# mjiUST/SurfaceNet

Hardware: AMD Instinct MI355X
Metric: voxel-cubes/sec (CVC warp + 3D CNN fwd) at s=32, N_viewpair=2 (higher is better)
Workload: dtype f16x3 (each operand = hi+lo fp16 pair, 3 MFMAs per product, f32 accumulate: fp32-class results; the two correction terms of a product run on one MX-scaled MFMA in the two merge layers (fp6 e2m3 codes) and in the three dilated layers conv4_x (fp8 e4m3 codes); L_inf vs fp64 oracle 3e-5 .. 1.7e-4, asse; 1 GPU; synthetic 2-view 1600x1200, s=32, batch=64 cubes/GPU, N_viewpair=2 (BASELINE.json configs[1]); cubes_per_gpu=64, parallelism=cube-sharded x1

## Files before the change

surfacenet_amd/csrc/conv3d_mfma.h:

```cpp
#pragma once
#include <hip/hip_runtime.h>
#include "mx_format.h"
#include <stdint.h>
#include <type_traits>

constexpr int kRowGap3x3 = 4, kRowGap2D = 4, kRowGapDil2 = 2;
#ifndef SN_TIMING
#define SN_TIMING 0
#endif
#define PW_SB __builtin_amdgcn_sched_barrier(0)

namespace sn {

typedef _Float16 half8 __attribute__((ext_vector_type(8)));
typedef _Float16 half4 __attribute__((ext_vector_type(4)));
typedef float f32x4 __attribute__((ext_vector_type(4)));

constexpr int kMaxSlab = 128;

struct ConvArgs {
    const _Float16 *in;
    _Float16 *out;
    float *out_f32;
    const _Float16 *wpack;
// ... 154 lines not shown
    static constexpr int TX = F4 ? NW * MF : NW * XS, TY = F4 ? 4 : 8, TZ = F4 ? 4 : 8;
    static constexpr int HX = TX + 2 * RX, HY = TY + 2 * R, HZ = TZ + 2 * R;
    static constexpr int HVOX = HX * HY * HZ;
    static constexpr int CS8MAX = CS8;
    static constexpr int SLOTS = CS8 + PADV_;
    static constexpr int VS = SLOTS * 16;
    static constexpr int PCH = PCH_;
    static constexpr int NPL = SPLIT ? 2 : 1;
    static constexpr int NPLM = SPLIT == 1 ? 2 : 1;
    static constexpr int FRAG = 1024 * NPL;
    static constexpr int MFRAG = 1024 * NPLM;
    static_assert(SPLIT < 2 || PCH_ == 2, "f16m8: a weight piece is 2 K-chunks + one MX step");
    static constexpr int MXF = SPLIT == 3 ? 0 : SN_MX_FMT;
    static constexpr int WBUF = PCH * NF * FRAG;
    static constexpr int NTAP = (K2D ? 1 : KS) * KS * KS;
    static constexpr int KOFF_N = NTAP * CS8MAX + 24;
    static constexpr bool PWM = (SPLIT == 3 || (SPLIT == 2 && SN_MX_FMT != 0)) && K2D == 0 && NW_ == 4 && KS == 3 && MF == 8 && PCH_ == 2;
    static constexpr int PW_TABS = 16;
    static constexpr int pw_tab(int kb, int slab, bool last) { return kb * PW_TABS + (last ? 8 : 0) + (slab & 7); }
    static constexpr int pw_xoff(int m) { return (((m >> 2) * HY + (m & 3)) * HZ) * VS; }
    static constexpr int XGAP = DIL == 2 ? kRowGapDil2 : kRowGap3x3;
    static constexpr int xoff_of(int m) { return XGAP == 4 ? pw_xoff(m) : (((m >> 2) * HY + (m & 1) + 4 * ((m >> 1) & 1)) * HZ) * VS; }
    static constexpr bool PTAB = SPLIT < 2 && NW_ == 8 && KS == 3 && PCH_ >= 2 && (K2D == 0 || SPLIT != 0) && !PWM;
    static constexpr int KTAB_N = PWM ? PW_TABS * KOFF_N : (PTAB ? 8 * KOFF_N : KOFF_N);
    static constexpr int NSEG0 = (HVOX * VS + 1023) / 1024;
    static constexpr int NSEG = PWM ? (NSEG0 + NW_ - 1) / NW_ * NW_ : NSEG0;
    static constexpr int XPLANE = NSEG * 1024;
    static constexpr int XBUF = XPLANE * NPL;
#ifndef SN_PW_WB3
#define SN_PW_WB3 0
// ... 144 lines not shown
        static_for<0, HT>([&](auto kc) {
            constexpr int k = decltype(kc)::value;
            const int li = k * C::NW + wave;
            if ((k + 1 < HT || C::NSEG * NPL == HT * C::NW || li < C::NSEG * NPL) && k >= kb && k < ke) {
                const char *base = (NPL > 1 && li >= C::NSEG) ? base0 + 2 * a.in_lo_off : base0;
                const __amdgpu_buffer_rsrc_t rs = __builtin_amdgcn_make_buffer_rsrc((void *)base, (short)0, nrec, 0x00020000);
                dma16_buf(rs, (hword[k] & keep) + (unsigned)toff, xbuf + xb * C::XBUF + li * 1024);
                ++issued;
            }
        });
        return issued;
    };
    auto wg_barrier = [&]() { asm volatile("s_barrier" ::: "memory"); };
    constexpr bool BRIDGE_OK = (PPX && SPLIT == 1) || PPM || PWM;
    constexpr int UM = SPLIT >= 2 ? 8 : 4;
    constexpr int BSTEP = (UM - (C::NTAP * C::CS8MAX) % UM) % UM;
    const bool bridge = BRIDGE_OK && a.bridge != 0;
    auto slab_units = [&](int c8n, int slab, int &o, int &b) {
        const int GU = C::NTAP * c8n;
        o = 0; b = 0;
        if (bridge) {
            o = (slab * ((UM - (GU & (UM - 1))) & (UM - 1))) & (UM - 1);
            b = (slab + 1 == a.nslab) ? 0 : ((UM - ((GU - o) & (UM - 1))) & (UM - 1));
        }
        return GU - o + b;
    };
    auto chunks_of = [&](int c8n, int slab) { int o, b; return (slab_units(c8n, slab, o, b) + 3) >> 2; };
    auto wchunks_of = [&](int c8n, int slab) { int o, b; return SPLIT >= 2 ? (((slab_units(c8n, slab, o, b) + 7) >> 3) << 1) : chunks_of(c8n, slab); };
    const int wchunk0 = wchunks_of(slab_c8_of(0), 0);
    auto write_koff_part = [&](int c8n, int kb, int slab, int t0, int nt) {
        int uo, ub;
        const int own = slab_units(c8n, slab, uo, ub) - ub, nchunk = (own + ub + 3) >> 2;
        int *k = kbuf + (PWM ? C::pw_tab(kb, slab, slab + 1 == a.nslab) : (C::PTAB ? kb * 8 + ((slab + 1 == a.nslab) ? 4 : 0) + (slab & 3) : kb)) * C::KOFF_N;
        for (int g = t0; g < (nchunk + 4) * 4; g += nt) {
            int o = 0;
            if (g < own + ub) {
                const int u = g < own ? g + uo : g - own;
                const int far = g < own ? 0 : (1 - 2 * kb) * C::XBUF;
                const int tap = C::CS8MAX == 1 ? u : u / c8n, c8 = C::CS8MAX == 1 ? 0 : u - tap * c8n;
                const int dz = tap % KS, dy = (tap / KS) % KS, dx = tap / (KS * KS);
                o = ((dx * DIL * C::HY + dy * DIL) * C::HZ + dz * DIL) * C::VS + c8 * 16 + far;
            }
            k[g] = o;
        }
    };
    auto write_koff = [&](int c8n, int kb, int slab) { write_koff_part(c8n, kb, slab, tid, C::NT); };
    auto stage_w = [&](size_t off, int nch, int wbi) {
        const int cnt = nch * NF * NPL;
        const char *src = wsrc0 + off;
        char *dst = wbuf + wbi * C::WBUF;
        for (int i = wave; i < cnt; i += C::NW) dma16(src + (size_t)i * 1024 + lane * 16, dst + i * 1024);
    };

    constexpr bool PMAP = (EPI == EPI_SIDEPOOL);
    static_assert(!PMAP || ((MF == 4 || MF == 8) && NW_ == 8 && K2D == 0), "EPI_SIDEPOOL: 8 waves x 4 (8) fragments over an 8x8x8 (16x8x8) tile");
// ... 102 lines not shown
            const unsigned tab0 = kbuf_a + (unsigned)(C::pw_tab(xb, 0, a.nslab == 1) * (C::KOFF_N * 4));
            int koA;
            lds_read32<0>(koA, tab0);
            lds_read32<16>(pw_koB, tab0);
            lds_read64<0>(pw_k2, tab0 + kq * 4);
            lgkm_wait<0>();
            const unsigned xa = xbuf_a + xb * C::XBUF + (unsigned)xbase[0] + (unsigned)koA, wp0 = wbuf_a + wbi * C::WBUF;
            static_for<0, MF>([&](auto mc) { constexpr int m = decltype(mc)::value; lds_read128<C::xoff_of(m)>(pw_xf[m], xa); });
            static_for<0, NF>([&](auto nc) { constexpr int n = decltype(nc)::value; lds_read128<n * 1024>(pw_wf[n], wp0); });
            lgkm_wait<0>();
        }
        if constexpr (PWM) __builtin_assume(a.nslab >= 1);
        for (int slab = 0; slab < a.nslab; ++slab) {
            const bool last_slab = slab + 1 == a.nslab;
            const int c8n = last_slab ? a.c8_last : C::CS8MAX;
            const int su_o = sl_o, su_b = (UM - ((C::NTAP * c8n - su_o) & (UM - 1))) & ((bridge && !last_slab) ? UM - 1 : 0);
            const int units = C::NTAP * c8n - su_o + su_b;
            const int nchunk = (units + 3) >> 2, wchunk = SPLIT >= 2 ? ((units + 7) >> 3) << 1 : nchunk;
            const int npiece = (nchunk + C::PCH - 1) / C::PCH;
            const int ntile = last_slab ? tile + tstride : tile;
            const bool have_next = ntile < a.total_tiles;
            const int nslab_i = last_slab ? 0 : slab + 1;
            const bool nlast = nslab_i + 1 == a.nslab;
            const int nc8n = nlast ? a.c8_last : C::CS8MAX;
            const int n_o = (bridge && !last_slab) ? (su_o + BSTEP) & (UM - 1) : 0;
            const int n_units = C::NTAP * nc8n - n_o + ((UM - ((C::NTAP * nc8n - n_o) & (UM - 1))) & ((bridge && !nlast) ? UM - 1 : 0));
            const int n_wchunk = SPLIT >= 2 ? ((n_units + 7) >> 3) << 1 : (n_units + 3) >> 2;
            const int nc0 = last_slab ? 0 : c0 + c8n;
            const size_t nwoff = last_slab ? 0 : woff + (size_t)wchunk * NF * C::FRAG;
            if constexpr (!PP && !PWM) { if (have_next) write_koff(nc8n, xb ^ 1, nslab_i); }
            int hdone = 0;

            if constexpr (PWM) {
                static_assert(SPLIT >= 2 && C::PCH == 2 && BUFH && EPI != EPI_SIDEPOOL && C::NSEG % C::NW == 0 && C::XPLANE + C::xoff_of(MF - 1) < 65536,
                              "one-wave-per-SIMD loop: f16m8 3x3x3 kernels");
                long long pws1 = 0;
                constexpr int mxo = 2 * NF * 1024;
                constexpr int WCNT = C::PCH * NF * NPL, WPW = (WCNT + C::NW - 1) / C::NW;
                constexpr int NM = MF * NF;
                constexpr int DSP = (NM - 16) / (WPW + HT / 2) >= 3 ? 3 : 2;
                static_assert(MF + NF <= 16 && 16 + DSP * (WPW + HT / 2 - 1) < NM && 4 + 2 * NF + 15 < NM, "filler schedule exceeds the burst");
                const unsigned tab_a = kbuf_a + (unsigned)(C::pw_tab(xb, slab, last_slab) * (C::KOFF_N * 4));
// ... 167 lines not shown
            if constexpr (PPX) {
                static_assert(C::PCH >= 2 && BUFH && SPLIT < 2 && C::PTAB, "ping-pong loop (f16 / f16x3): at least two chunks per weight piece");
                const unsigned koff_a = kbuf_a + (unsigned)((xb * 8 + (last_slab ? 4 : 0) + (slab & 3)) * (C::KOFF_N * 4));
                const unsigned xslab = xbuf_a + xb * C::XBUF;
                constexpr int NPLM = C::NPLM;
                int ko, ko_n = 0;
                const int bridge_b = su_b;
                lds_read32<0>(ko, koff_a);
                lgkm_wait<0>();
                int p = 0;
                do {
                    const int ch0 = p * C::PCH;
                    const unsigned wp = wbuf_a + wbi * C::WBUF;
                    const int nseg = (nchunk - ch0) < C::PCH ? (nchunk - ch0) : C::PCH;
                    int hnow = 0;
                    static_for<0, C::PCH>([&](auto scc) {
                        constexpr int sc = decltype(scc)::value;
                        if (sc < nseg) {
                            half8 xf[NPLM][MF], wf[NPLM][NF];
                            {
                                const unsigned kos = xslab + (unsigned)ko;
                                constexpr bool XIMM = K2D == 0 && !PMAP && KS == 3 && C::XPLANE + C::xoff_of(MF - 1) < 65536;
                                const unsigned kos0 = (unsigned)xbase[0] + kos;
                                static_for<0, MF>([&](auto mc) {
                                    constexpr int m = decltype(mc)::value;
                                    if constexpr (XIMM) {
                                        lds_read128<C::xoff_of(m)>(xf[0][m], kos0);
                                        if constexpr (SPLIT == 1) lds_read128<C::XPLANE + C::xoff_of(m)>(xf[1][m], kos0);
                                    } else {
                                        lds_read128<0>(xf[0][m], (unsigned)xbase[m] + kos);
                                        if constexpr (SPLIT == 1) {
                                            if constexpr (C::XPLANE < 65536) lds_read128<(C::XPLANE < 65536 ? C::XPLANE : 0)>(xf[1][m], (unsigned)xbase[m] + kos);
                                            else lds_read128<0>(xf[1][m], (unsigned)xbase[m] + kos + C::XPLANE);
                                        }
                                    }
                                });
                                static_for<0, NF>([&](auto nc) {
                                    constexpr int n = decltype(nc)::value;
                                    lds_read128<(sc * NF + n) * C::MFRAG>(wf[0][n], wp);
                                    if constexpr (SPLIT == 1) lds_read128<(sc * NF + n) * C::MFRAG + 1024>(wf[1][n], wp);
                                });
                                lds_read32<0>(ko_n, koff_a + (unsigned)(ch0 + sc + 1) * 16);
                            }
                            if constexpr (sc == 0) {
                                const bool real = (p + 1 < npiece) || have_next;
                                const size_t w_off = (p + 1 < npiece) ? woff + (size_t)(ch0 + C::PCH) * NF * C::FRAG : nwoff;
                                int w_nch = C::PCH;
                                if (p + 1 < npiece) { const int rem = wchunk - (ch0 + C::PCH); if (rem < C::PCH) w_nch = rem; }
                                else { if (n_wchunk < C::PCH) w_nch = n_wchunk; }
                                const char *src = wsrc0 + (real ? w_off : 0);
                                char *dst = wbuf + (wbi ^ 1) * C::WBUF;
                                const int cnt = (real ? w_nch : (wchunk0 < C::PCH ? wchunk0 : C::PCH)) * NF * NPL;
                                constexpr int WPWX = (C::PCH * NF * NPL + C::NW - 1) / C::NW;
                                static_for<0, WPWX>([&](auto kc) {
                                    int i = decltype(kc)::value * C::NW + wave;
                                    i = i < cnt ? i : cnt - 1;
                                    dma16(src + (size_t)i * 1024 + lane * 16, dst + i * 1024);
                                });
                                if (p == 0 && have_next)
                                    hnow = stage_halo_buf(last_slab ? nxt_b : (K2D ? x0 : b), last_slab ? nxt_keep : cur_keep, last_slab ? nxt_toff : cur_toff, nc0, nc8n, xb ^ 1);
                            }
                            const bool pre_bridge = bridge_b > 0 && ch0 + sc == nchunk - 2;
                            if (sc == nseg - 1) {
                                if (!pre_bridge && p + 1 < npiece && hnow == HT) asm volatile("s_waitcnt vmcnt(%0)" ::"i"(HT) : "memory");
                                else if (!pre_bridge && p + 1 < npiece && HT > 1 && hnow == HT - 1) asm volatile("s_waitcnt vmcnt(%0)" ::"i"(HT > 1 ? HT - 1 : 0) : "memory");
                                else asm volatile("s_waitcnt vmcnt(0)" ::: "memory");
                            } else if (pre_bridge) asm volatile("s_waitcnt vmcnt(0)" ::: "memory");
                            lgkm_wait<0>();
                            ko = ko_n;
                            wg_barrier();
                            __builtin_amdgcn_sched_barrier(0);
#pragma unroll
                            for (int n = 0; n < NF; ++n) {
                                if constexpr (SPLIT == 1) {
#pragma unroll
                                    for (int m = 0; m < MF; ++m) acc[m][n] = __builtin_amdgcn_mfma_f32_16x16x32_f16(wf[1][n], xf[0][m], acc[m][n], 0, 0, 0);
#pragma unroll
                                    for (int m = 0; m < MF; ++m) acc[m][n] = __builtin_amdgcn_mfma_f32_16x16x32_f16(wf[0][n], xf[1][m], acc[m][n], 0, 0, 0);
                                }
#pragma unroll
                                for (int m = 0; m < MF; ++m) acc[m][n] = __builtin_amdgcn_mfma_f32_16x16x32_f16(wf[0][n], xf[0][m], acc[m][n], 0, 0, 0);
                            }
                            __builtin_amdgcn_sched_barrier(0);
                            wg_barrier();
// ... 665 lines not shown
```

surfacenet_amd/csrc/sn_api.hip:

```cpp
#include "sn_internal.h"

enum Kind { K_CONV3, K_CONV1, K_DIL3, K_DIL1, K_UP };
struct LayerSpec { const char *name; Kind kind; int cin, cout, act; const char *input; };
static const LayerSpec kSpecs[] = {
    {"conv1_1", K_CONV3, 6, 32, 0, nullptr},       {"conv1_2", K_CONV3, 32, 32, 0, "conv1_1"},    {"conv1_3", K_CONV3, 32, 32, 0, "conv1_2"},
    {"side_op1", K_CONV1, 32, 16, 1, "conv1_3"},
    {"conv2_1", K_CONV3, 32, 80, 0, "conv1_3"},    {"conv2_2", K_CONV3, 80, 80, 0, "conv2_1"},    {"conv2_3", K_CONV3, 80, 80, 0, "conv2_2"},
    {"side_op2", K_CONV1, 80, 16, 1, "conv2_3"},   {"side_op2_deconv", K_UP, 3, 2, 0, nullptr},
    {"conv3_1", K_CONV3, 80, 160, 0, "conv2_3"},   {"conv3_2", K_CONV3, 160, 160, 0, "conv3_1"},  {"conv3_3", K_CONV3, 160, 160, 0, "conv3_2"},
    {"side_op3", K_CONV1, 160, 16, 1, "conv3_3"},  {"side_op3_deconv", K_UP, 5, 4, 0, nullptr},
    {"conv4_1", K_DIL3, 160, 300, 0, "conv3_3"},   {"conv4_2", K_DIL3, 300, 300, 0, "conv4_1"},   {"conv4_3", K_DIL3, 300, 300, 0, "conv4_2"},
    {"side_op4", K_DIL1, 300, 16, 1, "conv4_3"},   {"side_op4_deconv", K_UP, 5, 4, 0, nullptr},
    {"merge_conv_a", K_CONV3, 64, 100, 0, nullptr}, {"merge_conv_b", K_CONV3, 100, 100, 0, "merge_conv_a"}, {"merge_conv3", K_CONV1, 100, 1, 1, "merge_conv_b"},
};
static constexpr int kNumSpecs = sizeof(kSpecs) / sizeof(kSpecs[0]);
static constexpr int kNetParams = 98, kAllParams = 105, kDFeature = 258, kHidden = 100;


static unsigned char fp8_e4m3(float v)
{
    if (v != v) return 0x7f;
    const unsigned char sgn = std::signbit(v) ? 0x80 : 0;
    float a = std::fabs(v);
    if (a >= 448.f) return sgn | 0x7e;
// ... 59 lines not shown
            for (size_t i = (size_t)o * L.cin * ntap; i < (size_t)(o + 1) * L.cin * ntap; ++i) Wn[i] = std::ldexp(Wn[i], row_exp[o]);
    }
    if (ntap == 1) L.w_norm = Wn;
    const float *W = Wn.data();
    auto wat = [&](int o, int c8abs, int j, int tap) -> float {
        const int ci = c8abs * 8 + j;
        return (o < L.cout && ci < L.cin) ? W[((size_t)o * L.cin + ci) * ntap + tap] : 0.f;
    };
    h.clear();
    {
        const int um = split >= 2 ? 8 : 4;
        bool ok = L.bridge && (split == 1 || (split >= 2 && !L.k2d)) && L.ks == 3 && L.slab_c8.size() >= 2 && (ntap * cs8max) % um != 0;
        for (unsigned char c8n : L.slab_c8) ok = ok && c8n == cs8max;
        L.bridge = ok ? 1 : 0;
    }
    const int nslab = (int)L.slab_c8.size();
    auto slab_units = [&](int si, int c8n, int &o, int &b) {
        const int GU = ntap * c8n, um = split >= 2 ? 8 : 4;
        o = 0; b = 0;
        if (L.bridge) { o = (si * ((um - GU % um) % um)) % um; b = (si + 1 == nslab) ? 0 : (um - (GU - o) % um) % um; }
        return GU - o + b;
    };
    if (split < 2) {
        long long chunks = 0;
        for (int si = 0; si < nslab; ++si) { int o, b; chunks += (slab_units(si, L.slab_c8[si], o, b) + 3) / 4; }
        L.wsplit_stride = chunks * nf * 512 * npl;
        h.assign((size_t)L.wsplit_stride * nsplit, (_Float16)0.f);
        for (int ns = 0; ns < nsplit; ++ns) {
            _Float16 *dst = h.data() + (size_t)ns * L.wsplit_stride;
            int c8_0 = 0;
            for (int si = 0; si < nslab; ++si) {
                const int c8n = L.slab_c8[si];
                int uo, ub;
                const int own = slab_units(si, c8n, uo, ub) - ub, nchunk = (own + ub + 3) / 4;
                for (int ch = 0; ch < nchunk; ++ch)
                    for (int f = 0; f < nf; ++f)
                        for (int lane = 0; lane < 64; ++lane) {
                            const int o = (ns * nf + f) * 16 + (lane & 15);
                            const int g = 4 * ch + (lane >> 4);
                            _Float16 *d8 = dst + (((size_t)ch * nf + f) * npl * 64 + lane) * 8;
                            if (g >= own + ub) continue;
                            const int u = g < own ? g + uo : g - own;
                            const int cb = g < own ? c8_0 : c8_0 + c8n;
                            for (int j = 0; j < 8; ++j) {
                                const float w = wat(o, cb + u % c8n, j, u / c8n);
                                const _Float16 hi = (_Float16)w;
                                d8[j] = hi;
                                if (split == 1) d8[512 + j] = (_Float16)(w - (float)hi);
                            }
                        }
                dst += (size_t)nchunk * nf * 512 * npl;
                c8_0 += c8n;
            }
        }
    } else {
        long long pieces = 0;
        for (int si = 0; si < nslab; ++si) { int o, b; pieces += (slab_units(si, L.slab_c8[si], o, b) + 7) / 8; }
        const size_t piece_halfs = (size_t)nf * 2048;
        L.wsplit_stride = pieces * piece_halfs;
        h.assign((size_t)L.wsplit_stride * nsplit, (_Float16)0.f);
// ... 85 lines not shown
        const int oe = out_exp ? out_exp[o] : 0;
        sc[o] = std::ldexp(s, oe - row_exp[o]);
        sh[o] = std::ldexp(beta[o] - mean[o] * s, oe);
        if (!std::isfinite(sc[o]) || !std::isfinite(sh[o]) || (s != 0.f && sc[o] == 0.f))
            return fail(SN_ERR_ARG, "%s: folded BatchNorm scale / shift of output channel %d leaves the fp32 range (gamma %g, inv_std %g, "
                                    "row exponent %d, output exponent %d)", L.name.c_str(), o, gamma[o], inv_std[o], row_exp[o], oe);
    }
    L.macs_per_voxel = (double)L.cin * L.cout * ntap;
    return SN_OK;
}

int pack_conv(sn_ctx *c, PackedConv &L, const ConvEntry &e, const float *W_in, const float *beta, const float *gamma, const float *mean,
              const float *inv_std, const int *in_exp, const int *out_exp)
{
    L = PackedConv();
    L.name = e.name; L.cin = e.cin; L.cout = e.cout; L.act = e.act; L.ks = e.k.ks; L.dil = e.k.dil; L.k2d = e.k.k2d; L.bridge = e.bridge;
    std::vector<_Float16> h;
    std::vector<float> sc, sh;
    int rc;
    if ((rc = pack_conv_host(L, W_in, beta, gamma, mean, inv_std, e.k.nf, e.k.nsplit(e.cout), e.k.cs8max, e.k.split, in_exp, out_exp, h, sc, sh)) != SN_OK) return rc;
    if ((rc = dev_alloc(c, &L.wpack, h.size() + 8192)) != SN_OK) return rc;
    if ((rc = dev_alloc(c, &L.scale, sc.size())) != SN_OK) return rc;
    if ((rc = dev_alloc(c, &L.shift, sh.size())) != SN_OK) return rc;
    HIPCHK(hipMemcpy(L.wpack, h.data(), h.size() * sizeof(_Float16), hipMemcpyHostToDevice));
    HIPCHK(hipMemcpy(L.scale, sc.data(), sc.size() * sizeof(float), hipMemcpyHostToDevice));
    HIPCHK(hipMemcpy(L.shift, sh.data(), sh.size() * sizeof(float), hipMemcpyHostToDevice));
    return SN_OK;
}

static int pack_side_frag(sn_ctx *c, PackedConv &S, int producer_nf)
{
// ... 46 lines not shown
enum Tensor : unsigned char { T_NONE, T_X0, T_A1, T_B1, T_CAT, T_P1, T_A2, T_B2, T_S2, T_P2, T_A3, T_B3, T_A4, T_B4, T_S3, T_S4, T_MA, T_A3_HLC, T_A3_HC, T_COUNT };
static const TensorSpec kTensors[T_COUNT] = {
    {nullptr, 0, 0, MX_ACT, 0},      {&sn_ctx::x0, 0, 8, MX_X0, 0},    {&sn_ctx::a1, 0, 32, MX_ACT, 0},  {&sn_ctx::b1, 0, 32, MX_ACT, 0},  {&sn_ctx::cat, 0, 64, MX_CAT, 0},
    {&sn_ctx::p1, 1, 32, MX_ACT, 0}, {&sn_ctx::a2, 1, 80, MX_ACT, 0},  {&sn_ctx::b2, 1, 80, MX_ACT, 0},  {&sn_ctx::s2, 1, 16, MX_ACT, 0},  {&sn_ctx::p2, 2, 80, MX_ACT, 0},
    {&sn_ctx::a3, 2, 160, MX_ACT, 0}, {&sn_ctx::b3, 2, 160, MX_ACT, 0}, {&sn_ctx::a4, 2, 304, MX_ACT, 0}, {&sn_ctx::b4, 2, 304, MX_ACT, 0}, {&sn_ctx::s3, 2, 16, MX_ACT, 0},
    {&sn_ctx::s4, 2, 16, MX_ACT, 0}, {&sn_ctx::ma, 0, 104, MX_ACT, 0}, {&sn_ctx::a3, 2, 160, MX_ACT, 1}, {&sn_ctx::a3, 2, 160, MX_ACT, 2},
};

template <int SP>
static NetPlan build_plan_t(int tail_m8, int c4_m8)
{
    constexpr int PCH = SP == 2 ? 2 : 4;
    using Conv1 = ConvKernel<3, 1, 8, 2, EPI_STORE, SP, 1, PCH, 8, 0>;
    using Side = ConvKernel<1, 1, 4, 1, EPI_STORE, SP, 5, 2, 4, 0>;
    using Conv23 = ConvKernel<3, 1, 4, 5, EPI_STORE, SP, 1, PCH, 8, 0>;
    using Conv4 = ConvKernel<3, 2, 4, 5, EPI_STORE, SP, 1, 2, 8, 0>;
    static const bool unfused = sn_ab_switch("SN_NO_EPI_FUSION") != nullptr;
    static const bool no_bridge = sn_ab_switch("SN_NO_BRIDGE") != nullptr;
    NetPlan p{SP, tail_m8, c4_m8, {}, {kTensors, kTensors + T_COUNT}, launch_pool<SP>, launch_up3<SP>};
    ConvGeom conv1_3 = ConvKernel<3, 1, 4, 2, EPI_SIDEPOOL, SP, 1, (SP == 2 ? 2 : 7), 8, 0>::geom, side_op1 = Side::geom, conv3_3 = Conv23::geom,
             conv4_1 = Conv4::geom, conv4_2 = conv4_1, conv4_3 = conv4_1,
             merge_a = ConvKernel<3, 1, 4, 7, EPI_STORE, SP, (SP == 0 ? 2 : 1), (SP == 0 ? 4 : 2), 8, 0>::geom,
             merge_b = ConvKernel<3, 1, 4, 7, EPI_FINAL, SP, 1, (SP == 0 ? 4 : 2), 8, 0>::geom;
    Tensor conv3_3_out = T_A3, conv4_1_in = T_A3;
    if constexpr (SP == 1) {
        if (tail_m8 >= 2) {
            conv1_3 = ConvKernel<3, 1, 8, 2, EPI_SIDEPOOL, 1, 1, 4, 8, 0, 0, 2>::geom;
            side_op1 = ConvKernel<1, 1, 4, 1, EPI_STORE, 1, 5, 2, 4, 0, 0, 2>::geom;
            p.up3 = launch_up3<1, 2>;
            merge_a = ConvKernel<3, 1, 8, 7, EPI_STORE, 2, 1, 2, 4, 0>::geom;
            merge_b = ConvKernel<3, 1, 8, 7, EPI_FINAL, 2, 1, 2, 4, 0>::geom;
        }
        if (c4_m8) {
            conv4_1 = conv4_2 = ConvKernel<3, 2, 8, 5, EPI_STORE, 3, 1, 2, 4, 0>::geom;
            conv4_3 = ConvKernel<3, 2, 8, 5, EPI_STORE, 3, 1, 2, 4, 0, 0, 1>::geom;
            if (c4_m8 == 2) conv4_1 = ConvKernel<3, 2, 4, 5, EPI_STORE, 1, 1, 2, 8, 0, 0, 3>::geom;
            else { conv3_3 = ConvKernel<3, 1, 4, 5, EPI_STORE, 1, 1, 4, 8, 0, 0, 4>::geom; conv3_3_out = T_A3_HLC; conv4_1_in = T_A3_HC; }
            for (Tensor t : {T_A3, T_A3_HLC, T_A3_HC, T_A4, T_B4}) p.tens[t].e8 = MX_C4;
        }
    }
    auto add = [&](const char *name, ConvGeom k, Tensor in, Tensor out, Tensor pool_out = T_NONE, const char *pool_tag = nullptr) -> ConvEntry & {
        ConvEntry e{name, 0, 0, 0, k, (k.has_bridge && !no_bridge) ? 1 : 0, in, out, pool_out, pool_tag};
        for (const LayerSpec &sp : kSpecs) if (!strcmp(sp.name, name)) { e.cin = sp.cin; e.cout = sp.cout; e.act = sp.act; }
        p.conv.push_back(e);
        return p.conv.back();
    };
    add("conv1_1", Conv1::geom, T_X0, T_A1);
    add("conv1_2", Conv1::geom, T_A1, T_B1);
    add("conv1_3", unfused ? Conv1::geom : conv1_3, T_B1, unfused ? T_A1 : T_NONE);
    add("side_op1", side_op1, T_A1, T_CAT, T_P1, "pool1");
    add("conv2_1", Conv23::geom, T_P1, T_A2);
    add("conv2_2", Conv23::geom, T_A2, T_B2);
    add("conv2_3", unfused ? Conv23::geom : ConvKernel<3, 1, 4, 5, EPI_SIDEPOOL, SP, 1, PCH, 8, 0>::geom, T_B2, unfused ? T_A2 : T_NONE);
    add("side_op2", Side::geom, T_A2, T_S2, T_P2, "pool2");
    add("conv3_1", Conv23::geom, T_P2, T_A3);
    add("conv3_2", Conv23::geom, T_A3, T_B3);
    add("conv3_3", conv3_3, T_B3, conv3_3_out);
    add("side_op3", Side::geom, T_A3, T_S3);
    add("conv4_1", conv4_1, conv4_1_in, T_A4);
    add("conv4_2", conv4_2, T_A4, T_B4);
    add("conv4_3", conv4_3, T_B4, T_A4);
    add("side_op4", Side::geom, T_A4, T_S4).up3 = true;
    add("merge_conv_a", merge_a, T_CAT, T_MA);
    add("merge_conv_b", merge_b, T_MA, T_NONE);
    return p;
}

static NetPlan build_plan(int split, int tail_m8, int c4_m8)
{
    return split == 2 ? build_plan_t<2>(tail_m8, c4_m8) : (split == 1 ? build_plan_t<1>(tail_m8, c4_m8) : build_plan_t<0>(tail_m8, c4_m8));
}
// ... 1062 lines not shown
    if (bytes > (size_t)info[6]) return fail(SN_ERR_ARG, "sn_debug_tensor: %s holds %lld bytes, %zu asked for", name, info[6], bytes);
    const _Float16 *p = d.a3c ? c->a3c : c->*kTensors[d.buf].buf;
    const size_t own = d.a3c || d.fmt != 4 ? bytes : std::min(bytes, (size_t)info[4] * 2);
    HIPCHK(hipSetDevice(c->device));
    HIPCHK(hipStreamSynchronize(c->stream));
    HIPCHK(hipMemcpy(host, p, own, hipMemcpyDeviceToHost));
    if (bytes > own) HIPCHK(hipMemcpy(static_cast<char *>(host) + own, c->a3c, bytes - own, hipMemcpyDeviceToHost));
    return SN_OK;
}

SN_API int sn_debug_pack_host(int cin, int cout, int ks, int dil, int k2d, int nf, int nsplit, int cs8max, int split, const float *W, const float *beta,
                              const float *gamma, const float *mean, const float *inv_std, unsigned long long *out)
{
    if (!W || !beta || !gamma || !mean || !inv_std || !out) return fail(SN_ERR_ARG, "null argument");
    PackedConv L;
    L.name = "debug"; L.cin = cin; L.cout = cout; L.ks = ks; L.dil = dil; L.k2d = k2d;
    L.bridge = 1;
    std::vector<_Float16> h;
    std::vector<float> sc, sh;
    const int rc = pack_conv_host(L, W, beta, gamma, mean, inv_std, nf, nsplit, cs8max, split, nullptr, nullptr, h, sc, sh);
    if (rc != SN_OK) return rc;
    unsigned long long sum = 0;
    const unsigned char *b = reinterpret_cast<const unsigned char *>(h.data());
    for (size_t i = 0; i < h.size() * sizeof(_Float16); ++i) sum = sum * 1099511628211ull + b[i];
    out[0] = h.size(); out[1] = sc.size(); out[2] = sh.size(); out[3] = sum;
    return SN_OK;
}

SN_API int sn_debug_plan(int net, int mode, int conv4_fp8, char *rows, int cap)
{
    if (!rows || cap < 1 || net < 0 || net > 1) return fail(SN_ERR_ARG, "sn_debug_plan: bad argument");
    sn_ctx st;
    int rc = sn_set_precision(&st, mode), n = 0;
    if (rc == SN_OK && conv4_fp8 >= 0) rc = sn_set_conv4_fp8(&st, conv4_fp8);
    if (rc != SN_OK) return rc;
    for (const ConvEntry &e : net == 0 ? build_plan(st.split, st.tail_m8, st.c4_m8).conv : simil_plan(st.split)) {
        n += snprintf(rows + n, (size_t)(cap - n), "%s %d %d %d %d %d %d %d %d %d %d %d %d\n", e.name, e.cin, e.cout, e.k.ks, e.k.dil, e.k.k2d,
                      e.k.nf, e.k.nsplit(e.cout), e.k.cs8max, e.k.split, e.k.osplit, e.k.epi, e.bridge);
        if (n >= cap) return fail(SN_ERR_ARG, "sn_debug_plan: the rows do not fit %d bytes", cap);
    }
    return SN_OK;
}

SN_API int sn_debug_mx6_encode(float v, int fmt) { return (fmt == 2 || fmt == 3) ? (int)mx6_encode(v, fmt) : -1; }

SN_API int sn_debug_timing(sn_ctx *c, unsigned long long *out, int n_layers, char *names, int names_cap)
{
    if (!c || !out || !c->d_num) return fail(SN_ERR_ARG, "null argument");
    HIPCHK(hipStreamSynchronize(c->stream));
    n_layers = std::min(n_layers, 32);
    HIPCHK(hipMemcpy(out, c->d_num + 2, sizeof(unsigned long long) * 4 * n_layers, hipMemcpyDeviceToHost));
    HIPCHK(hipMemset(c->d_num + 2, 0, sizeof(unsigned) * 32 * 8));
    std::string all;
// ... 51 lines not shown
```

surfacenet_amd/csrc/sn_internal.h:

```cpp
#pragma once
#include <hip/hip_runtime.h>
#include <dlfcn.h>

#include <algorithm>
#include <chrono>
#include <cmath>
#include <condition_variable>
#include <memory>
#include <mutex>
#include <thread>
#include <type_traits>
#include <cstring>
#include <map>
#include <string>
#include <vector>

#include "sn_host.h"
#include "conv3d_mfma.h"
#include "cvc_warp.h"
#include "elementwise.h"

using namespace sn;

#define HIPCHK(expr)                                                                                       \
    do {                                                                                                   \
        hipError_t e_ = (expr);                                                                            \
        if (e_ != hipSuccess) return fail(SN_ERR_HIP, "%s failed: %s (%s:%d)", #expr, hipGetErrorString(e_), __FILE__, __LINE__); \
    } while (0)

struct PackedConv {
    std::string name;
    int cin = 0, cout = 0, ks = 1, dil = 1, act = 0;
    int cin_p = 0;
    int nf = 0, nsplit = 1;
    int cs8max = 4, split = 0, k2d = 0;
    int bridge = 0;
    std::vector<unsigned char> slab_c8;
    long long wsplit_stride = 0;
    _Float16 *wpack = nullptr;
    float *scale = nullptr, *shift = nullptr;
    double macs_per_voxel = 0;
    std::vector<float> w_norm;
    _Float16 *side_frag = nullptr;
};

struct sn_ctx;
enum MxExp : unsigned char { MX_ACT, MX_CAT, MX_X0, MX_C4 };

struct Act { _Float16 *p; long long lo; long long code = 0; MxExp e8 = MX_ACT; };

struct SideFuse { const PackedConv *side; Act side_out; int side_cs, side_coff; Act pool_out; int pool_cs; };

struct ConvGeom {
    int ks, dil, k2d, nf, cs8max, split, osplit, epi;
    bool has_bridge;
    int (*launch)(sn_ctx *c, const PackedConv &L, Act in, int in_cs, Act out, int out_cs, int out_coff, int out_cp, float *out_f32, int B, int D, int DX, const SideFuse *sf);
    int nsplit(int cout) const { return ((cout + 15) / 16 + nf - 1) / nf; }
};

struct ConvEntry {
    const char *name; int cin, cout, act;
    ConvGeom k;
    int bridge;
    unsigned char in = 0, out = 0, pool_out = 0;
    const char *pool_tag = nullptr;
    bool up3 = false;
};
struct TensorSpec { _Float16 *sn_ctx::*buf; int level, ch; MxExp e8; int code; };
struct NetPlan {
    int split = -1, tail_m8 = 0, c4_m8 = 0;
// ... 249 lines not shown
            if (it == c->num_names.end() && c->num_names.size() < 31) c->num_names.push_back(L.name);
            a.status = c->d_num;
            constexpr int OS = OSPLIT < 0 ? SPLIT : OSPLIT;
            if (EPI == EPI_STORE && OS >= 2 && L.act == 0) {
                const _Float16 lim = (_Float16)std::min(60000.f, std::ldexp(OS >= 3 ? 255.875f : (SN_MX_FMT == 2 ? 7.5f : 28.f), a.mx_out_e8 - 127));
                unsigned short bits; memcpy(&bits, &lim, 2);
                a.mx_sat_bits = bits;
            }
            a.status_bit = bit < 31 ? (1u << bit) : (1u << 31);
        }
        a.nslab = (int)L.slab_c8.size();
        if (a.nslab < 1) return fail(SN_ERR_STATE, "%s: no channel slabs", L.name.c_str());
        a.bridge = L.bridge;
        if (L.bridge && !geom.has_bridge)
            return fail(SN_ERR_STATE, "%s: packed with bridge chunks, launched on a kernel without them", L.name.c_str());
        if (C::PWM) {
            for (unsigned char c8n : L.slab_c8)
                if (C::NTAP * c8n < 9) return fail(SN_ERR_STATE, "%s: a channel slab of fewer than two weight pieces", L.name.c_str());
        }
        for (int i = 0; i + 1 < a.nslab; ++i)
            if (L.slab_c8[i] != C::CS8MAX) return fail(SN_ERR_STATE, "%s: channel slab %d holds %d groups, the kernel expects %d in all but the last", L.name.c_str(), i, (int)L.slab_c8[i], C::CS8MAX);
        a.c8_last = L.slab_c8.back();
        const double vox = (double)B * DX * D * D;
        const double bytes = vox * 2.0 * (SPLIT ? 2 : 1) * (L.cin + (EPI == EPI_FINAL ? 2 : (EPI == EPI_SIDEPOOL ? 16 + L.cout / 8.0 : L.cout)));
        ProfScope ps(c, L.name, 2.0 * L.macs_per_voxel * vox, bytes);
        const int resident = std::max(1, c->num_cus * C::WG_PER_CU / L.nsplit);
        dim3 grid((unsigned)std::min(a.total_tiles, resident), (unsigned)L.nsplit);
        hipLaunchKernelGGL((conv3d_f16_mfma<KS, DIL, MF, NF, EPI, SPLIT, CS8, PCH, NW, PADV, K2D, OSPLIT>), grid, dim3(NW * 64), 0, c->stream, a);
        HIPCHK(hipGetLastError());
        return SN_OK;
    }
    static constexpr ConvGeom geom = {KS, DIL, K2D != 0, NF, C::CS8MAX, SPLIT, OSPLIT < 0 ? SPLIT : OSPLIT, EPI,
                                      sn::sn_conv_has_bridge<KS, SPLIT, NW, PCH, NF, K2D, MF>(), &launch};
};

struct TmpDev {
    std::vector<void *> p;
    bool ok = true;
    ~TmpDev() { for (void *q : p) (void)hipFree(q); }
    template <typename T> T *out(size_t count)
    {
        void *q = nullptr;
        if (hipMalloc(&q, std::max<size_t>(count, 1) * sizeof(T)) != hipSuccess) { ok = false; return nullptr; }
        p.push_back(q);
        return static_cast<T *>(q);
    }
    template <typename T> T *up(sn_ctx *c, const T *host, size_t count)
    {
// ... 6 lines not shown
```

Measured before the change: 7412 cubes/s.

## Reorder K stream into tap triples to reuse activation fragments across shifted taps

For split-f16 3x3x3 convs with one 8-channel group per slab, the weight stream is reordered so each piece covers three taps along one axis. The kernel loads the activation register window once per triple and reuses shifted fragments across the three taps instead of re-reading LDS for each tap. The offset table and weight packing are rewritten to match, with a launch-time check that packing order equals kernel order. This trades fewer LDS reads for more registers holding the window (rp array) and 3-chunk pieces.

```diff
diff --git a/surfacenet_amd/csrc/conv3d_mfma.h b/surfacenet_amd/csrc/conv3d_mfma.h
--- a/surfacenet_amd/csrc/conv3d_mfma.h
+++ b/surfacenet_amd/csrc/conv3d_mfma.h
@@ -192,6 +192,10 @@
     static constexpr int MXF = SPLIT == 3 ? 0 : SN_MX_FMT;
     static constexpr int WBUF = PCH * NF * FRAG;
     static constexpr int NTAP = (K2D ? 1 : KS) * KS * KS;
+    static constexpr bool TRI = SPLIT == 1 && NW_ == 8 && KS == 3 && DIL == 1 && K2D == 0 && CS8 == 1 && PCH_ == 3;
+    static constexpr int KORDER = !TRI ? 0 : (EPI == 3  ? 2 : 1);
+    static constexpr int UPG = TRI ? NTAP / 3 : NTAP;
+    static constexpr int CPQ = TRI ? 3 : 1;
     static constexpr int KOFF_N = NTAP * CS8MAX + 24;
     static constexpr bool PWM = (SPLIT == 3 || (SPLIT == 2 && SN_MX_FMT != 0)) && K2D == 0 && NW_ == 4 && KS == 3 && MF == 8 && PCH_ == 2;
     static constexpr int PW_TABS = 16;
@@ -366,10 +370,10 @@
     auto wg_barrier = [&]() { asm volatile("s_barrier" ::: "memory"); };
     constexpr bool BRIDGE_OK = (PPX && SPLIT == 1) || PPM || PWM;
     constexpr int UM = SPLIT >= 2 ? 8 : 4;
-    constexpr int BSTEP = (UM - (C::NTAP * C::CS8MAX) % UM) % UM;
+    constexpr int BSTEP = (UM - (C::UPG * C::CS8MAX) % UM) % UM;
     const bool bridge = BRIDGE_OK && a.bridge != 0;
     auto slab_units = [&](int c8n, int slab, int &o, int &b) {
-        const int GU = C::NTAP * c8n;
+        const int GU = C::UPG * c8n;
         o = 0; b = 0;
         if (bridge) {
             o = (slab * ((UM - (GU & (UM - 1))) & (UM - 1))) & (UM - 1);
@@ -377,7 +381,7 @@
         }
         return GU - o + b;
     };
-    auto chunks_of = [&](int c8n, int slab) { int o, b; return (slab_units(c8n, slab, o, b) + 3) >> 2; };
+    auto chunks_of = [&](int c8n, int slab) { int o, b; return ((slab_units(c8n, slab, o, b) + 3) >> 2) * C::CPQ; };
     auto wchunks_of = [&](int c8n, int slab) { int o, b; return SPLIT >= 2 ? (((slab_units(c8n, slab, o, b) + 7) >> 3) << 1) : chunks_of(c8n, slab); };
     const int wchunk0 = wchunks_of(slab_c8_of(0), 0);
     auto write_koff_part = [&](int c8n, int kb, int slab, int t0, int nt) {
@@ -390,7 +394,9 @@
                 const int u = g < own ? g + uo : g - own;
                 const int far = g < own ? 0 : (1 - 2 * kb) * C::XBUF;
                 const int tap = C::CS8MAX == 1 ? u : u / c8n, c8 = C::CS8MAX == 1 ? 0 : u - tap * c8n;
-                const int dz = tap % KS, dy = (tap / KS) % KS, dx = tap / (KS * KS);
+                int dz = tap % KS, dy = (tap / KS) % KS, dx = tap / (KS * KS);
+                if constexpr (C::KORDER == 1) { dx = u / KS; dy = 0; dz = u % KS; }
+                if constexpr (C::KORDER == 2) { dx = 0; dy = u / KS; dz = u % KS; }
                 o = ((dx * DIL * C::HY + dy * DIL) * C::HZ + dz * DIL) * C::VS + c8 * 16 + far;
             }
             k[g] = o;
@@ -523,9 +529,9 @@
         for (int slab = 0; slab < a.nslab; ++slab) {
             const bool last_slab = slab + 1 == a.nslab;
             const int c8n = last_slab ? a.c8_last : C::CS8MAX;
-            const int su_o = sl_o, su_b = (UM - ((C::NTAP * c8n - su_o) & (UM - 1))) & ((bridge && !last_slab) ? UM - 1 : 0);
-            const int units = C::NTAP * c8n - su_o + su_b;
-            const int nchunk = (units + 3) >> 2, wchunk = SPLIT >= 2 ? ((units + 7) >> 3) << 1 : nchunk;
+            const int su_o = sl_o, su_b = (UM - ((C::UPG * c8n - su_o) & (UM - 1))) & ((bridge && !last_slab) ? UM - 1 : 0);
+            const int units = C::UPG * c8n - su_o + su_b;
+            const int nchunk = ((units + 3) >> 2) * C::CPQ, wchunk = SPLIT >= 2 ? ((units + 7) >> 3) << 1 : nchunk;
             const int npiece = (nchunk + C::PCH - 1) / C::PCH;
             const int ntile = last_slab ? tile + tstride : tile;
             const bool have_next = ntile < a.total_tiles;
@@ -533,8 +539,8 @@
             const bool nlast = nslab_i + 1 == a.nslab;
             const int nc8n = nlast ? a.c8_last : C::CS8MAX;
             const int n_o = (bridge && !last_slab) ? (su_o + BSTEP) & (UM - 1) : 0;
-            const int n_units = C::NTAP * nc8n - n_o + ((UM - ((C::NTAP * nc8n - n_o) & (UM - 1))) & ((bridge && !nlast) ? UM - 1 : 0));
-            const int n_wchunk = SPLIT >= 2 ? ((n_units + 7) >> 3) << 1 : (n_units + 3) >> 2;
+            const int n_units = C::UPG * nc8n - n_o + ((UM - ((C::UPG * nc8n - n_o) & (UM - 1))) & ((bridge && !nlast) ? UM - 1 : 0));
+            const int n_wchunk = SPLIT >= 2 ? ((n_units + 7) >> 3) << 1 : ((n_units + 3) >> 2) * C::CPQ;
             const int nc0 = last_slab ? 0 : c0 + c8n;
             const size_t nwoff = last_slab ? 0 : woff + (size_t)wchunk * NF * C::FRAG;
             if constexpr (!PP && !PWM) { if (have_next) write_koff(nc8n, xb ^ 1, nslab_i); }
@@ -732,12 +738,28 @@
                     const unsigned wp = wbuf_a + wbi * C::WBUF;
                     const int nseg = (nchunk - ch0) < C::PCH ? (nchunk - ch0) : C::PCH;
                     int hnow = 0;
+                    constexpr bool TRI = C::TRI;
+                    constexpr int NP = PMAP ? MF / 2 : 4, NC = MF / NP;
+                    constexpr int AXS = (PMAP ? C::HY * C::HZ : C::HZ) * C::VS, CLS = (PMAP ? C::HZ : C::HY * C::HZ) * C::VS;
+                    static_assert(!TRI || (C::PCH == 3 && C::XPLANE + (NC - 1) * CLS + (NP + 1) * AXS < 65536), "triple order: 3-chunk pieces, immediate offsets");
+                    half8 rp[TRI ? NPLM : 1][TRI ? NC : 1][TRI ? NP + 2 : 1];
                     static_for<0, C::PCH>([&](auto scc) {
                         constexpr int sc = decltype(scc)::value;
-                        if (sc < nseg) {
+                        if (TRI || sc < nseg) {
                             half8 xf[NPLM][MF], wf[NPLM][NF];
                             {
                                 const unsigned kos = xslab + (unsigned)ko;
+                                if constexpr (TRI) {
+                                    const unsigned kos0 = (unsigned)xbase[0] + kos;
+                                    static_for<0, MF>([&](auto mc) {
+                                        constexpr int m = decltype(mc)::value, c = PMAP ? (m & 1) : (m >> 2), q = PMAP ? (m >> 1) : (m & 3);
+                                        constexpr int qn = sc == 0 ? q : NP - 1 + sc;
+                                        if constexpr (sc == 0 || q == 0) {
+                                            lds_read128<c * CLS + qn * AXS>(rp[0][c][qn], kos0);
+                                            lds_read128<C::XPLANE + c * CLS + qn * AXS>(rp[1][c][qn], kos0);
+                                        }
+                                    });
+                                } else {
                                 constexpr bool XIMM = K2D == 0 && !PMAP && KS == 3 && C::XPLANE + C::xoff_of(MF - 1) < 65536;
                                 const unsigned kos0 = (unsigned)xbase[0] + kos;
                                 static_for<0, MF>([&](auto mc) {
@@ -753,12 +775,14 @@
                                         }
                                     }
                                 });
+                                }
                                 static_for<0, NF>([&](auto nc) {
                                     constexpr int n = decltype(nc)::value;
                                     lds_read128<(sc * NF + n) * C::MFRAG>(wf[0][n], wp);
                                     if constexpr (SPLIT == 1) lds_read128<(sc * NF + n) * C::MFRAG + 1024>(wf[1][n], wp);
                                 });
-                                lds_read32<0>(ko_n, koff_a + (unsigned)(ch0 + sc + 1) * 16);
+                                if constexpr (!TRI) lds_read32<0>(ko_n, koff_a + (unsigned)(ch0 + sc + 1) * 16);
+                                else if constexpr (sc == C::PCH - 1) lds_read32<0>(ko_n, koff_a + (unsigned)(p + 1) * 16);
                             }
                             if constexpr (sc == 0) {
                                 const bool real = (p + 1 < npiece) || have_next;
@@ -778,14 +802,19 @@
                                 if (p == 0 && have_next)
                                     hnow = stage_halo_buf(last_slab ? nxt_b : (K2D ? x0 : b), last_slab ? nxt_keep : cur_keep, last_slab ? nxt_toff : cur_toff, nc0, nc8n, xb ^ 1);
                             }
-                            const bool pre_bridge = bridge_b > 0 && ch0 + sc == nchunk - 2;
+                            const bool pre_bridge = bridge_b > 0 && ch0 + sc == nchunk - (TRI ? 4 : 2);
                             if (sc == nseg - 1) {
                                 if (!pre_bridge && p + 1 < npiece && hnow == HT) asm volatile("s_waitcnt vmcnt(%0)" ::"i"(HT) : "memory");
                                 else if (!pre_bridge && p + 1 < npiece && HT > 1 && hnow == HT - 1) asm volatile("s_waitcnt vmcnt(%0)" ::"i"(HT > 1 ? HT - 1 : 0) : "memory");
                                 else asm volatile("s_waitcnt vmcnt(0)" ::: "memory");
                             } else if (pre_bridge) asm volatile("s_waitcnt vmcnt(0)" ::: "memory");
                             lgkm_wait<0>();
-                            ko = ko_n;
+                            if constexpr (!TRI || sc == C::PCH - 1) ko = ko_n;
+                            if constexpr (TRI)
+                                static_for<0, MF>([&](auto mc) {
+                                    constexpr int m = decltype(mc)::value, c = PMAP ? (m & 1) : (m >> 2), q = PMAP ? (m >> 1) : (m & 3);
+                                    xf[0][m] = rp[0][c][q + sc]; xf[NPLM - 1][m] = rp[NPLM - 1][c][q + sc];
+                                });
                             wg_barrier();
                             __builtin_amdgcn_sched_barrier(0);
 #pragma unroll
diff --git a/surfacenet_amd/csrc/sn_api.hip b/surfacenet_amd/csrc/sn_api.hip
--- a/surfacenet_amd/csrc/sn_api.hip
+++ b/surfacenet_amd/csrc/sn_api.hip
@@ -97,16 +97,21 @@
         for (unsigned char c8n : L.slab_c8) ok = ok && c8n == cs8max;
         L.bridge = ok ? 1 : 0;
     }
+    {
+        bool ok = (L.korder == 1 || L.korder == 2) && split == 1 && L.ks == 3 && !L.k2d && L.dil == 1 && cs8max == 1;
+        L.korder = ok ? L.korder : 0;
+    }
+    const int tri = L.korder, upg = tri ? ntap / 3 : ntap, cpq = tri ? 3 : 1;
     const int nslab = (int)L.slab_c8.size();
     auto slab_units = [&](int si, int c8n, int &o, int &b) {
-        const int GU = ntap * c8n, um = split >= 2 ? 8 : 4;
+        const int GU = upg * c8n, um = split >= 2 ? 8 : 4;
         o = 0; b = 0;
         if (L.bridge) { o = (si * ((um - GU % um) % um)) % um; b = (si + 1 == nslab) ? 0 : (um - (GU - o) % um) % um; }
         return GU - o + b;
     };
     if (split < 2) {
         long long chunks = 0;
-        for (int si = 0; si < nslab; ++si) { int o, b; chunks += (slab_units(si, L.slab_c8[si], o, b) + 3) / 4; }
+        for (int si = 0; si < nslab; ++si) { int o, b; chunks += (slab_units(si, L.slab_c8[si], o, b) + 3) / 4 * cpq; }
         L.wsplit_stride = chunks * nf * 512 * npl;
         h.assign((size_t)L.wsplit_stride * nsplit, (_Float16)0.f);
         for (int ns = 0; ns < nsplit; ++ns) {
@@ -115,18 +120,19 @@
             for (int si = 0; si < nslab; ++si) {
                 const int c8n = L.slab_c8[si];
                 int uo, ub;
-                const int own = slab_units(si, c8n, uo, ub) - ub, nchunk = (own + ub + 3) / 4;
+                const int own = slab_units(si, c8n, uo, ub) - ub, nchunk = (own + ub + 3) / 4 * cpq;
                 for (int ch = 0; ch < nchunk; ++ch)
                     for (int f = 0; f < nf; ++f)
                         for (int lane = 0; lane < 64; ++lane) {
                             const int o = (ns * nf + f) * 16 + (lane & 15);
-                            const int g = 4 * ch + (lane >> 4);
+                            const int g = 4 * (ch / cpq) + (lane >> 4), t = ch % cpq;
                             _Float16 *d8 = dst + (((size_t)ch * nf + f) * npl * 64 + lane) * 8;
                             if (g >= own + ub) continue;
                             const int u = g < own ? g + uo : g - own;
                             const int cb = g < own ? c8_0 : c8_0 + c8n;
                             for (int j = 0; j < 8; ++j) {
-                                const float w = wat(o, cb + u % c8n, j, u / c8n);
+                                const int tap = tri == 1 ? (u / 3) * 9 + t * 3 + u % 3 : (tri == 2 ? t * 9 + u : u / c8n);
+                                const float w = wat(o, cb + u % c8n, j, tap);
                                 const _Float16 hi = (_Float16)w;
                                 d8[j] = hi;
                                 if (split == 1) d8[512 + j] = (_Float16)(w - (float)hi);
@@ -242,7 +248,7 @@
               const float *inv_std, const int *in_exp, const int *out_exp)
 {
     L = PackedConv();
-    L.name = e.name; L.cin = e.cin; L.cout = e.cout; L.act = e.act; L.ks = e.k.ks; L.dil = e.k.dil; L.k2d = e.k.k2d; L.bridge = e.bridge;
+    L.name = e.name; L.cin = e.cin; L.cout = e.cout; L.act = e.act; L.ks = e.k.ks; L.dil = e.k.dil; L.k2d = e.k.k2d; L.bridge = e.bridge; L.korder = e.k.korder;
     std::vector<_Float16> h;
     std::vector<float> sc, sh;
     int rc;
@@ -319,11 +325,16 @@
     using Conv1 = ConvKernel<3, 1, 8, 2, EPI_STORE, SP, 1, PCH, 8, 0>;
     using Side = ConvKernel<1, 1, 4, 1, EPI_STORE, SP, 5, 2, 4, 0>;
     using Conv23 = ConvKernel<3, 1, 4, 5, EPI_STORE, SP, 1, PCH, 8, 0>;
+    constexpr int TPCH = SP == 1 ? 3 : PCH;
+    using Conv1T = ConvKernel<3, 1, 8, 2, EPI_STORE, SP, 1, TPCH, 8, 0>;
+    using Conv23T = ConvKernel<3, 1, 4, 5, EPI_STORE, SP, 1, TPCH, 8, 0>;
+    using Conv23PoolT = ConvKernel<3, 1, 4, 5, EPI_SIDEPOOL, SP, 1, TPCH, 8, 0>;
+    const bool tri = SP == 1 && tail_m8 < 2;
     using Conv4 = ConvKernel<3, 2, 4, 5, EPI_STORE, SP, 1, 2, 8, 0>;
     static const bool unfused = sn_ab_switch("SN_NO_EPI_FUSION") != nullptr;
     static const bool no_bridge = sn_ab_switch("SN_NO_BRIDGE") != nullptr;
     NetPlan p{SP, tail_m8, c4_m8, {}, {kTensors, kTensors + T_COUNT}, launch_pool<SP>, launch_up3<SP>};
-    ConvGeom conv1_3 = ConvKernel<3, 1, 4, 2, EPI_SIDEPOOL, SP, 1, (SP == 2 ? 2 : 7), 8, 0>::geom, side_op1 = Side::geom, conv3_3 = Conv23::geom,
+    ConvGeom conv1_3 = ConvKernel<3, 1, 4, 2, EPI_SIDEPOOL, SP, 1, (SP == 2 ? 2 : 7), 8, 0>::geom, side_op1 = Side::geom, conv3_3 = tri ? Conv23T::geom : Conv23::geom,
              conv4_1 = Conv4::geom, conv4_2 = conv4_1, conv4_3 = conv4_1,
              merge_a = ConvKernel<3, 1, 4, 7, EPI_STORE, SP, (SP == 0 ? 2 : 1), (SP == 0 ? 4 : 2), 8, 0>::geom,
              merge_b = ConvKernel<3, 1, 4, 7, EPI_FINAL, SP, 1, (SP == 0 ? 4 : 2), 8, 0>::geom;
@@ -351,15 +362,15 @@
         return p.conv.back();
     };
     add("conv1_1", Conv1::geom, T_X0, T_A1);
-    add("conv1_2", Conv1::geom, T_A1, T_B1);
+    add("conv1_2", tri ? Conv1T::geom : Conv1::geom, T_A1, T_B1);
     add("conv1_3", unfused ? Conv1::geom : conv1_3, T_B1, unfused ? T_A1 : T_NONE);
     add("side_op1", side_op1, T_A1, T_CAT, T_P1, "pool1");
-    add("conv2_1", Conv23::geom, T_P1, T_A2);
-    add("conv2_2", Conv23::geom, T_A2, T_B2);
-    add("conv2_3", unfused ? Conv23::geom : ConvKernel<3, 1, 4, 5, EPI_SIDEPOOL, SP, 1, PCH, 8, 0>::geom, T_B2, unfused ? T_A2 : T_NONE);
+    add("conv2_1", tri ? Conv23T::geom : Conv23::geom, T_P1, T_A2);
+    add("conv2_2", tri ? Conv23T::geom : Conv23::geom, T_A2, T_B2);
+    add("conv2_3", unfused ? Conv23::geom : (tri ? Conv23PoolT::geom : ConvKernel<3, 1, 4, 5, EPI_SIDEPOOL, SP, 1, PCH, 8, 0>::geom), T_B2, unfused ? T_A2 : T_NONE);
     add("side_op2", Side::geom, T_A2, T_S2, T_P2, "pool2");
-    add("conv3_1", Conv23::geom, T_P2, T_A3);
-    add("conv3_2", Conv23::geom, T_A3, T_B3);
+    add("conv3_1", tri ? Conv23T::geom : Conv23::geom, T_P2, T_A3);
+    add("conv3_2", tri ? Conv23T::geom : Conv23::geom, T_A3, T_B3);
     add("conv3_3", conv3_3, T_B3, conv3_3_out);
     add("side_op3", Side::geom, T_A3, T_S3);
     add("conv4_1", conv4_1, conv4_1_in, T_A4);
@@ -1452,7 +1463,8 @@
 {
     if (!W || !beta || !gamma || !mean || !inv_std || !out) return fail(SN_ERR_ARG, "null argument");
     PackedConv L;
-    L.name = "debug"; L.cin = cin; L.cout = cout; L.ks = ks; L.dil = dil; L.k2d = k2d;
+    L.name = "debug"; L.cin = cin; L.cout = cout; L.ks = ks; L.dil = dil; L.k2d = k2d & 0xff;
+    L.korder = (k2d >> 8) & 3;
     L.bridge = 1;
     std::vector<_Float16> h;
     std::vector<float> sc, sh;
@@ -1467,14 +1479,18 @@
 
 SN_API int sn_debug_plan(int net, int mode, int conv4_fp8, char *rows, int cap)
 {
-    if (!rows || cap < 1 || net < 0 || net > 1) return fail(SN_ERR_ARG, "sn_debug_plan: bad argument");
+    if (!rows || cap < 1 || net < 0 || net > 3) return fail(SN_ERR_ARG, "sn_debug_plan: bad argument");
+    const bool with_korder = net >= 2;
+    net &= 1;
     sn_ctx st;
     int rc = sn_set_precision(&st, mode), n = 0;
     if (rc == SN_OK && conv4_fp8 >= 0) rc = sn_set_conv4_fp8(&st, conv4_fp8);
     if (rc != SN_OK) return rc;
     for (const ConvEntry &e : net == 0 ? build_plan(st.split, st.tail_m8, st.c4_m8).conv : simil_plan(st.split)) {
-        n += snprintf(rows + n, (size_t)(cap - n), "%s %d %d %d %d %d %d %d %d %d %d %d %d\n", e.name, e.cin, e.cout, e.k.ks, e.k.dil, e.k.k2d,
+        n += snprintf(rows + n, (size_t)(cap - n), "%s %d %d %d %d %d %d %d %d %d %d %d %d", e.name, e.cin, e.cout, e.k.ks, e.k.dil, e.k.k2d,
                       e.k.nf, e.k.nsplit(e.cout), e.k.cs8max, e.k.split, e.k.osplit, e.k.epi, e.bridge);
+        if (with_korder && n < cap) n += snprintf(rows + n, (size_t)(cap - n), " %d", e.k.korder);
+        if (n < cap) n += snprintf(rows + n, (size_t)(cap - n), "\n");
         if (n >= cap) return fail(SN_ERR_ARG, "sn_debug_plan: the rows do not fit %d bytes", cap);
     }
     return SN_OK;
diff --git a/surfacenet_amd/csrc/sn_internal.h b/surfacenet_amd/csrc/sn_internal.h
--- a/surfacenet_amd/csrc/sn_internal.h
+++ b/surfacenet_amd/csrc/sn_internal.h
@@ -35,6 +35,7 @@
     int nf = 0, nsplit = 1;
     int cs8max = 4, split = 0, k2d = 0;
     int bridge = 0;
+    int korder = 0;
     std::vector<unsigned char> slab_c8;
     long long wsplit_stride = 0;
     _Float16 *wpack = nullptr;
@@ -54,6 +55,7 @@
 struct ConvGeom {
     int ks, dil, k2d, nf, cs8max, split, osplit, epi;
     bool has_bridge;
+    int korder;
     int (*launch)(sn_ctx *c, const PackedConv &L, Act in, int in_cs, Act out, int out_cs, int out_coff, int out_cp, float *out_f32, int B, int D, int DX, const SideFuse *sf);
     int nsplit(int cout) const { return ((cout + 15) / 16 + nf - 1) / nf; }
 };
@@ -333,6 +335,8 @@
         a.bridge = L.bridge;
         if (L.bridge && !geom.has_bridge)
             return fail(SN_ERR_STATE, "%s: packed with bridge chunks, launched on a kernel without them", L.name.c_str());
+        if (L.korder != C::KORDER)
+            return fail(SN_ERR_STATE, "%s: weight stream in K order %d, the kernel runs order %d", L.name.c_str(), L.korder, C::KORDER);
         if (C::PWM) {
             for (unsigned char c8n : L.slab_c8)
                 if (C::NTAP * c8n < 9) return fail(SN_ERR_STATE, "%s: a channel slab of fewer than two weight pieces", L.name.c_str());
@@ -350,7 +354,7 @@
         return SN_OK;
     }
     static constexpr ConvGeom geom = {KS, DIL, K2D != 0, NF, C::CS8MAX, SPLIT, OSPLIT < 0 ? SPLIT : OSPLIT, EPI,
-                                      sn::sn_conv_has_bridge<KS, SPLIT, NW, PCH, NF, K2D, MF>(), &launch};
+                                      sn::sn_conv_has_bridge<KS, SPLIT, NW, PCH, NF, K2D, MF>(), C::KORDER, &launch};
 };
 
 struct TmpDev {
```

Result: no change. 7388 cubes/s (-0.3%).
